# amaciarey/PathIntegralGroundState

Hardware: AMD Instinct MI355X
Metric: bead-pair action evals/sec (K1 Delta-S, N=256 Nb=161 4He, 128 walkers/GPU) (higher is better)
Workload: dtype f64; 1 GPU; liquid 4He N=256 beads=161 (namelist Nb=80), 128 walkers/GPU x 1 GPU(s) = 128 walkers, one full-chain Delta-S stage per step (20608 items x 255 partners per GPU); walkers_per_gpu=128, global_walkers=128

## Files before the change

### pathintegralgroundstate_amd/csrc/pigs_device.h

```cpp
#pragma once

#include <hip/hip_runtime.h>
#include <stdint.h>

namespace pigs {

constexpr int kWave = 64;

struct DevParams {
    int32_t dim, Np, NpPad, Nb;
    int32_t M, Nmax, trap, wf_table;
    int32_t v_table, nW, pad1, pad2;
    double  dr, rcut2, dt, Rm;
    double  Lbox[3], LboxHalf[3], a_ho[3];
    double  rdr;
    double  hrdr;
    double  rLbox[3];
};

__host__ __device__ inline size_t slice_doubles(int dim, int NpPad) { return (size_t)dim * NpPad; }

__device__ __forceinline__ double wave_sum(double v)
{
#pragma unroll
    for (int off = 32; off >= 1; off >>= 1) v += __shfl_xor(v, off, kWave);
    return v;
}

template <int DIM>
__device__ __forceinline__ double min_image(double (&x)[DIM], const DevParams &P)
{
    double r2 = 0.0;
#pragma unroll
    for (int k = 0; k < DIM; ++k) {
        double v = x[k];
        if (v >  P.LboxHalf[k]) v = v - P.Lbox[k];
        if (v < -P.LboxHalf[k]) v = v + P.Lbox[k];
        x[k] = v;
        r2 = r2 + v * v;
    }
    return r2;
}

template <int DIM>
__device__ __forceinline__ double plain_r2(const double (&x)[DIM])
{
    double r2 = 0.0;
#pragma unroll
    for (int k = 0; k < DIM; ++k) r2 = r2 + x[k] * x[k];
    return r2;
}

struct Lerp {
    int    ix;
    int    im2;
    double a1, a2;
};

__device__ __forceinline__ Lerp lerp_setup(double x, double dx, int Nmax)
{
    Lerp L;
    int ix = (int)(x / dx) + 1;
    L.a1   = x - (double)(ix - 1) * dx;
    L.a2   = dx - L.a1;
    L.ix   = min(ix, Nmax);
    L.im2  = max(L.ix - 2, 0);
    return L;
}

__device__ __forceinline__ double interp0(const double *__restrict__ F, const Lerp &L, double dx)
{
    return (L.a1 * F[L.ix] + L.a2 * F[L.ix - 1]) / dx;
}

__device__ __forceinline__ double interp1(const double *__restrict__ F, const Lerp &L, double dx)
{
    double Fbefore = (L.a1 * F[L.ix - 1] + L.a2 * F[L.im2]) / dx;
    double Fafter  = (L.a1 * F[L.ix + 1] + L.a2 * F[L.ix]) / dx;
    return 0.5 * (Fafter - Fbefore) / dx;
}

__device__ __forceinline__ double interp2(const double *__restrict__ F, const Lerp &L, double dx)
{
    double Fbefore = (L.a1 * F[L.ix - 1] + L.a2 * F[L.im2]) / dx;
    double Fcurr   = (L.a1 * F[L.ix] + L.a2 * F[L.ix - 1]) / dx;
    double Fafter  = (L.a1 * F[L.ix + 1] + L.a2 * F[L.ix]) / dx;
    return (Fafter - 2.0 * Fcurr + Fbefore) / (dx * dx);
}

__device__ __forceinline__ double div_by(double a, double d, double rd)
{
    const double q = a * rd;
    const double r = __builtin_fma(-q, d, a);
    return __builtin_fma(r, rd, q);
}

__device__ __forceinline__ double div_by_inf(double a, double d, double rd)
{
    const double q = a * rd;
    const double r = __builtin_fma(-q, d, a);
    const double z = __builtin_fma(r, rd, q);
    return __builtin_fabs(q) == __builtin_inf() ? q : z;
}

__device__ __forceinline__ void sqrt_rinv(double x, double &s, double &y)
{
    const double y0 = __builtin_amdgcn_rsq(x);
    double g = x * y0;
    double h = 0.5 * y0;
    const double r0 = __builtin_fma(-h, g, 0.5);
    g = __builtin_fma(g, r0, g);
    h = __builtin_fma(h, r0, h);
    const double d0 = __builtin_fma(-g, g, x);
    g = __builtin_fma(d0, h, g);
    const double d1 = __builtin_fma(-g, g, x);
    g = __builtin_fma(d1, h, g);
    s = g;
    double yy = h + h;
    const double e = __builtin_fma(-g, yy, 1.0);
    y = __builtin_fma(e, yy, yy);
}

__device__ __forceinline__ double sqrt_exact(double x)
{
    double s, y;
    sqrt_rinv(x, s, y);
    return s;
}

struct FLerp {
    int    ix, im2;
    double a1, a2;
};

__device__ __forceinline__ FLerp flerp_setup(double x, const DevParams &P)
{
    FLerp L;
    const int ix = (int)div_by(x, P.dr, P.rdr) + 1;
    L.a1  = x - (double)(ix - 1) * P.dr;
    L.a2  = P.dr - L.a1;
    L.ix  = min(ix, P.Nmax);
#ifdef PIGS_EXPERIMENT_HOT_TABLE
    L.ix  = (L.ix & 63) + 2;
#endif
    L.im2 = max(L.ix - 2, 0);
    return L;
}

template <typename TabPtr>
__device__ __forceinline__ double finterp0(TabPtr F, const FLerp &L, const DevParams &P)
{
    return div_by_inf(L.a1 * F[L.ix] + L.a2 * F[L.ix - 1], P.dr, P.rdr);
}

template <typename TabPtr>
__device__ __forceinline__ void finterp01(TabPtr F, const FLerp &L, const DevParams &P, double &v0, double &v1)
{
    const double fm2 = F[L.im2], fm1 = F[L.ix - 1], f0 = F[L.ix], fp1 = F[L.ix + 1];
    v0 = div_by_inf(L.a1 * f0 + L.a2 * fm1, P.dr, P.rdr);
    const double Fbefore = div_by_inf(L.a1 * fm1 + L.a2 * fm2, P.dr, P.rdr);
    const double Fafter  = div_by_inf(L.a1 * fp1 + L.a2 * f0, P.dr, P.rdr);
    v1 = div_by_inf(0.5 * (Fafter - Fbefore), P.dr, P.rdr);
}

template <int DIM>
__device__ __forceinline__ double min_image_fast(double (&x)[DIM], const DevParams &P)
{
    double r2 = 0.0;
#pragma unroll
    for (int k = 0; k < DIM; ++k) {
        const double v = x[k];
        const double w = v - __builtin_copysign(P.Lbox[k], v);
        const double u = (__builtin_fabs(v) > P.LboxHalf[k]) ? w : v;
        x[k] = u;
        r2 = r2 + u * u;
    }
    return r2;
}

struct FastTab {
    const double *p;
    __device__ __forceinline__ double operator[](int i) const { return p[i]; }
};
template <typename T> struct is_fast_tab { static constexpr bool value = false; };
template <> struct is_fast_tab<FastTab> { static constexpr bool value = true; };

template <int DIM>
__device__ __forceinline__ double min_image_rn(double (&x)[DIM], const DevParams &P)
{
    double r2 = 0.0;
#pragma unroll
    for (int k = 0; k < DIM; ++k) {
        const double v = x[k];
        const double t = __builtin_fmin(__builtin_fmax(__builtin_fabs(v) * P.rLbox[k], 0.0), 1.0);
        const double n = __builtin_copysign(__builtin_rint(t), v);
        const double u = __builtin_fma(-P.Lbox[k], n, v);
        x[k] = u;
        r2 = r2 + u * u;
    }
    return r2;
}

template <int DIM>
__device__ __forceinline__ double min_image_mag(const double (&x)[DIM], const DevParams &P)
{
    double r2 = 0.0;
#pragma unroll
    for (int k = 0; k < DIM; ++k) {
        const double a = __builtin_fabs(x[k]);
        const double m = __builtin_fmin(a, P.Lbox[k] - a);
        r2 = r2 + m * m;
    }
    return r2;
}

struct FCell {
    int    i0;
    double f, omf;
    double r, rinv;
};

__device__ __forceinline__ FCell fcell_setup(double r2, const DevParams &P)
{
    FCell C;
    const double y0 = __builtin_amdgcn_rsq(r2);
    double g = r2 * y0;
    double h = 0.5 * y0;
    const double r0 = __builtin_fma(-h, g, 0.5);
    g = __builtin_fma(g, r0, g);
    h = __builtin_fma(h, r0, h);
    const double d0 = __builtin_fma(-g, g, r2);
    g = __builtin_fma(d0, h, g);
    C.r    = g;
    C.rinv = h + h;
    const double t = g * P.rdr;
    C.i0  = (int)t;
    C.f   = t - (double)C.i0;
    C.omf = 1.0 - C.f;
    return C;
}

template <int N>
__device__ __forceinline__ void wave_reduce_multi(double (&v)[N], int lane)
{
    int stride = 32;
#pragma unroll
    for (int cnt = N; cnt > 1; cnt >>= 1, stride >>= 1) {
        const bool upper = (lane & stride) != 0;
#pragma unroll
        for (int i = 0; i < cnt / 2; ++i) {
            const double send = upper ? v[i] : v[i + cnt / 2];
            const double keep = upper ? v[i + cnt / 2] : v[i];
            v[i] = keep + __shfl_xor(send, stride, kWave);
        }
    }
#pragma unroll
    for (; stride >= 1; stride >>= 1) v[0] += __shfl_xor(v[0], stride, kWave);
}

constexpr int kRedStride = 65;

template <int N>
__device__ __forceinline__ double wave_reduce_lds(const double (&v)[N], double *scratch, int lane)
{
    static_assert(N == 2 || N == 4 || N == 8, "N must divide 64");
#pragma unroll
    for (int i = 0; i < N; ++i) scratch[i * kRedStride + lane] = v[i];
    __builtin_amdgcn_wave_barrier();
    const int vi = lane % N, g = lane / N;
    const double *row = scratch + vi * kRedStride + g * N;
    double s = row[0];
#pragma unroll
    for (int k = 1; k < N; ++k) s = s + row[k];
    __builtin_amdgcn_wave_barrier();
#pragma unroll
    for (int stride = N; stride < kWave; stride <<= 1) s = s + __shfl_xor(s, stride, kWave);
    return s;
}

template <int N>
__device__ __forceinline__ constexpr int lane_of(int i)
{
    int lane = 0, stride = 32;
    for (int cnt = N; cnt > 1; cnt >>= 1, stride >>= 1)
        if (i & (cnt >> 1)) lane |= stride;
    return lane;
}

__device__ __forceinline__ double read_lane(double v, int lane)
{
    union { double d; int i[2]; } u;
    u.d = v;
    u.i[0] = __builtin_amdgcn_readlane(u.i[0], lane);
    u.i[1] = __builtin_amdgcn_readlane(u.i[1], lane);
    return u.d;
}

template <int N>
__device__ __forceinline__ double row_shl(double x)
{
    union { double d; int i[2]; } u, r;
    u.d = x;
    r.i[0] = __builtin_amdgcn_update_dpp(0, u.i[0], 0x100 + N, 0xf, 0xf, true);
    r.i[1] = __builtin_amdgcn_update_dpp(0, u.i[1], 0x100 + N, 0xf, 0xf, true);
    return r.d;
}

__host__ __device__ inline double green_function(int opt, int ib, int Nb, double dt, double Pot, double F2)
{
    double g = 0.0;
    if (opt == 0) {
        double Ve = Pot;
        double Vc = Pot + dt * dt * F2 / 6.0;
        if (ib == 0 || ib == 2 * Nb) g = dt * Ve / 3.0;
        else if ((ib & 1) == 0)      g = 2.0 * dt * Ve / 3.0;
        else                         g = 4.0 * dt * Vc / 3.0;
    } else {
        double dVe = Pot;
        double dVc = Pot + dt * dt * F2 / 2.0;
        if (ib == 0 || ib == 2 * Nb) g = dVe / 3.0;
        else if ((ib & 1) == 0)      g = 2.0 * dVe / 3.0;
        else                         g = 4.0 * dVc / 3.0;
    }
    return g;
}

__device__ __forceinline__ double green_function_action(int ib, int Nb, double dt_in, double Pot, double F2)
{
    constexpr double r3 = 1.0 / 3.0, r6 = 1.0 / 6.0;
    double dt = dt_in;
    asm volatile("" : "+v"(dt));
    if (ib == 0 || ib == 2 * Nb) return div_by_inf(dt * Pot, 3.0, r3);
    if ((ib & 1) == 0)           return div_by_inf(2.0 * dt * Pot, 3.0, r3);
    const double Vc = Pot + div_by_inf(dt * dt * F2, 6.0, r6);
    return div_by_inf(4.0 * dt * Vc, 3.0, r3);
}

__host__ __device__ inline double log_psi(int opt, double Rm, double r)
{
    const double q = Rm / r;
    const double q5 = q * q * q * q * q;
    if (opt == 0) return -0.5 * q5;
    if (opt == 1) return 2.5 * q5 / r;
    return -15.0 * q5 / (r * r);
}

__host__ __device__ inline double trap_pot(int opt, double a, double x)
{
    const double a4 = a * a * a * a;
    return opt == 0 ? 0.5 * (x * x) / a4 : x / a4;
}

__host__ __device__ inline double trap_psi(int opt, double a, double x)
{
    if (opt == 0) { double q = x / a; return -0.5 * (q * q); }
    if (opt == 1) return -(x / (a * a));
    return -1.0 / (a * a);
}

}
```

### pathintegralgroundstate_amd/csrc/pigs_k1.hip

```cpp
#include <atomic>

#include "pigs_device.h"
#include "pigs_k1_device.h"
#include "pigs_kernels.h"

namespace pigs {

template <int DIM, bool TRAP>
__global__ __launch_bounds__(256) void k_delta_action_v1(
    DevParams P, const double *__restrict__ paths, const double *__restrict__ VT,
    const double *__restrict__ WF, int n_items, const int32_t *__restrict__ walker,
    const int32_t *__restrict__ ipv, const int32_t *__restrict__ ibv,
    const double *__restrict__ xnew, const double *__restrict__ xold,
    double *__restrict__ out, double *__restrict__ parts)
{
    const int lane  = threadIdx.x & (kWave - 1);
    const int wid   = threadIdx.x >> 6;
    const int nwave = gridDim.x * (blockDim.x >> 6);
    const size_t sl = slice_doubles(DIM, P.NpPad);

    for (int item = blockIdx.x * (blockDim.x >> 6) + wid; item < n_items; item += nwave) {
        const int it = __builtin_amdgcn_readfirstlane(item);
        const int w  = walker[it];
        const int p  = ipv[it] - 1;
        const int b  = ibv[it];
        if ((unsigned)w >= (unsigned)P.nW || (unsigned)p >= (unsigned)P.Np || (unsigned)b >= (unsigned)P.M) {
            if (lane == 0) out[it] = __builtin_nan("");
            continue;
        }
        double xn[DIM], xo[DIM];
#pragma unroll
        for (int k = 0; k < DIM; ++k) {
            xn[k] = xnew[(size_t)it * DIM + k];
            xo[k] = xold[(size_t)it * DIM + k];
        }
        const double *S   = paths + ((size_t)w * P.M + b) * sl;
        const bool odd    = (b & 1) != 0;
        const bool endb   = (b == 0) || (b == 2 * P.Nb);

        double potN = 0.0, potO = 0.0, psiN = 0.0, psiO = 0.0;
        double fN[DIM], fO[DIM];
#pragma unroll
        for (int k = 0; k < DIM; ++k) { fN[k] = 0.0; fO[k] = 0.0; }

        if (TRAP && lane == 0) {
#pragma unroll
            for (int k = 0; k < DIM; ++k) {
                potN = potN + trap_pot(0, P.a_ho[k], xn[k]);
                potO = potO + trap_pot(0, P.a_ho[k], xo[k]);
                fO[k] = trap_pot(1, P.a_ho[k], xo[k]);
                fN[k] = trap_pot(1, P.a_ho[k], xn[k]);
                if (endb) {
                    psiO = psiO + trap_psi(0, P.a_ho[k], xo[k]);
                    psiN = psiN + trap_psi(0, P.a_ho[k], xn[k]);
                }
            }
        }

        for (int j0 = 0; j0 < P.Np; j0 += kWave) {
            const int j = j0 + lane;
            if (j < P.Np && j != p) {
                double dnew[DIM], dold[DIM];
#pragma unroll
                for (int k = 0; k < DIM; ++k) {
                    const double rj = S[(size_t)k * P.NpPad + j];
                    dnew[k] = xn[k] - rj;
                    dold[k] = xo[k] - rj;
                }
                double r2n, r2o;
                if (TRAP) { r2o = plain_r2<DIM>(dold); r2n = plain_r2<DIM>(dnew); }
                else      { r2o = min_image<DIM>(dold, P); r2n = min_image<DIM>(dnew, P); }

                if (TRAP || r2n <= P.rcut2) {
                    const double r = sqrt(r2n);
                    const Lerp L = lerp_setup(r, P.dr, P.Nmax);
                    potN = potN + interp0(VT, L, P.dr);
                    if (odd) {
                        const double dv = interp1(VT, L, P.dr);
#pragma unroll
                        for (int k = 0; k < DIM; ++k) fN[k] = fN[k] + dv * dnew[k] / r;
                    }
                    if (endb) psiN = psiN + (P.wf_table ? interp0(WF, L, P.dr) : log_psi(0, P.Rm, r));
                }
                if (r2o <= P.rcut2) {
                    const double r = sqrt(r2o);
                    const Lerp L = lerp_setup(r, P.dr, P.Nmax);
                    potO = potO + interp0(VT, L, P.dr);
                    if (odd) {
                        const double dv = interp1(VT, L, P.dr);
#pragma unroll
                        for (int k = 0; k < DIM; ++k) fO[k] = fO[k] + dv * dold[k] / r;
                    }
                    if (endb) psiO = psiO + (P.wf_table ? interp0(WF, L, P.dr) : log_psi(0, P.Rm, r));
                } else if (TRAP && endb) {
                    const double r = sqrt(r2o);
                    const Lerp L = lerp_setup(r, P.dr, P.Nmax);
                    psiO = psiO + (P.wf_table ? interp0(WF, L, P.dr) : log_psi(0, P.Rm, r));
                }
            }
        }

        potN = wave_sum(potN);
        potO = wave_sum(potO);
        double dF2 = 0.0, dPsi = 0.0;
        if (odd) {
            double fn2 = 0.0, fo2 = 0.0;
#pragma unroll
            for (int k = 0; k < DIM; ++k) {
                const double a = wave_sum(fN[k]);
                const double c = wave_sum(fO[k]);
                fn2 = fn2 + a * a;
                fo2 = fo2 + c * c;
            }
            dF2 = fn2 - fo2;
        }
        if (endb) {
            psiN = wave_sum(psiN);
            psiO = wave_sum(psiO);
            dPsi = psiN - psiO;
        }
        if (lane == 0) {
            const double dPot = potN - potO;
            out[it] = -dPsi + green_function(0, b, P.Nb, P.dt, dPot, dF2);
            if (parts) {
                parts[(size_t)it * 3 + 0] = dPot;
                parts[(size_t)it * 3 + 1] = dF2;
                parts[(size_t)it * 3 + 2] = dPsi;
            }
        }
    }
}


template <int DIM, bool TRAP, int BLOCK, bool PREFETCH = false, bool FAST = false>
__global__ __launch_bounds__(BLOCK) void k_delta_action_v2(
    DevParams P, const double *__restrict__ paths, const double *__restrict__ VT,
    const double *__restrict__ WF, int n_items, const int32_t *__restrict__ walker,
    const int32_t *__restrict__ ipv, const int32_t *__restrict__ ibv,
    const double *__restrict__ xnew, const double *__restrict__ xold,
    double *__restrict__ out, double *__restrict__ parts)
{
    extern __shared__ __attribute__((aligned(16))) unsigned char smem[];
    const int lane  = threadIdx.x & (kWave - 1);
    const int wid   = threadIdx.x >> 6;
    const int nwave = gridDim.x * (BLOCK >> 6);
    const size_t sl = slice_doubles(DIM, P.NpPad);
    double *red = reinterpret_cast<double *>(smem + (size_t)wid * kWaveLds);

    for (int item = blockIdx.x * (BLOCK >> 6) + wid; item < n_items; item += nwave) {
        const int it = __builtin_amdgcn_readfirstlane(item);
        const int w  = walker[it];
        const int p  = ipv[it] - 1;
        const int b  = ibv[it];
        if ((unsigned)w >= (unsigned)P.nW || (unsigned)p >= (unsigned)P.Np || (unsigned)b >= (unsigned)P.M) {
            if (lane == 0) out[it] = __builtin_nan("");
            continue;
        }
        double xn[DIM], xo[DIM];
#pragma unroll
        for (int k = 0; k < DIM; ++k) {
            xn[k] = xnew[(size_t)it * DIM + k];
            xo[k] = xold[(size_t)it * DIM + k];
        }
        const double *S = paths + ((size_t)w * P.M + b) * sl;
        double *o = out + it;
        double *q = parts ? parts + (size_t)it * 3 : nullptr;
        if (FAST && !TRAP) {
            if (PREFETCH) item_eval_prefetch<DIM, TRAP>(P, FastTab{VT}, WF, S, p, b, xn, xo, lane, red, o, q);
            else          item_eval<DIM, TRAP>(P, FastTab{VT}, WF, S, p, b, xn, xo, lane, red, o, q);
        } else if (PREFETCH) {
            item_eval_prefetch<DIM, TRAP>(P, VT, WF, S, p, b, xn, xo, lane, red, o, q);
        } else {
            item_eval<DIM, TRAP>(P, VT, WF, S, p, b, xn, xo, lane, red, o, q);
        }
    }
}

template <int DIM>
__global__ __launch_bounds__(256) void k_delta_action_grid(
    DevParams P, const double *__restrict__ paths, const double *__restrict__ VTimg,
    const double *__restrict__ WF, int n_items, const int32_t *__restrict__ walker,
    const int32_t *__restrict__ ipv, const int32_t *__restrict__ ibv,
    const double *__restrict__ xnew, const double *__restrict__ xold,
    double *__restrict__ out, double *__restrict__ parts)
{
    extern __shared__ __attribute__((aligned(16))) unsigned char smem[];
    const int lane  = threadIdx.x & (kWave - 1);
    const int wid   = threadIdx.x >> 6;
    const int nwave = gridDim.x * 4;
    const size_t sl = slice_doubles(DIM, P.NpPad);
    double *red = reinterpret_cast<double *>(smem + (size_t)wid * kWaveLds);
    const PipeTab VT{VTimg + 2, P.Nmax + 3};

    for (int item = blockIdx.x * 4 + wid; item < n_items; item += nwave) {
        const int it = __builtin_amdgcn_readfirstlane(item);
        const int w  = walker[it];
        const int p  = ipv[it] - 1;
        const int b  = ibv[it];
        if ((unsigned)w >= (unsigned)P.nW || (unsigned)p >= (unsigned)P.Np || (unsigned)b >= (unsigned)P.M) {
            if (lane == 0) out[it] = __builtin_nan("");
            continue;
        }
        double xn[DIM], xo[DIM];
#pragma unroll
        for (int k = 0; k < DIM; ++k) {
            xn[k] = xnew[(size_t)it * DIM + k];
            xo[k] = xold[(size_t)it * DIM + k];
        }
        item_eval_pipe<DIM>(P, VT, WF, paths + ((size_t)w * P.M + b) * sl, p, b, xn, xo, lane, red, out + it,
                            parts ? parts + (size_t)it * 3 : nullptr);
    }
}

template <int DIM, bool TRAP, int CLS>
__device__ __forceinline__ void reforder_item(const DevParams &P, const double *__restrict__ VT, const double *__restrict__ WF,
                                              const double *__restrict__ S, int p, int b, const double (&xn)[DIM],
                                              const double (&xo)[DIM], int lane, double *T, double *out, double *parts)
{
    for (int j = lane; j < P.Np; j += kWave) {
        Acc<DIM, CLS> A;
        if (j != p) {
            double rj[DIM];
#pragma unroll
            for (int k = 0; k < DIM; ++k) rj[k] = S[(size_t)k * P.NpPad + j];
            partner_accumulate_at<DIM, TRAP, CLS>(P, VT, WF, rj, xn, xo, A);
        }
        double *t = T + (size_t)j * 8;
        t[0] = A.potN; t[1] = A.potO;
        if (CLS == CLS_ODD) {
#pragma unroll
            for (int k = 0; k < DIM; ++k) { t[2 + k] = A.fN[k]; t[5 + k] = A.fO[k]; }
        } else if (CLS == CLS_END) {
            t[2] = A.psiN; t[3] = A.psiO;
        }
    }
    __builtin_amdgcn_wave_barrier();
    __syncthreads();
    double s = 0.0;
    if (lane < 8) {
        if (TRAP) {
            Acc<DIM, CLS> A0;
            trap_terms<DIM, TRAP, CLS>(P, xn, xo, A0);
            double col[8] = {A0.potN, A0.potO, 0.0, 0.0, 0.0, 0.0, 0.0, 0.0};
            if (CLS == CLS_ODD) {
#pragma unroll
                for (int k = 0; k < DIM; ++k) { col[2 + k] = A0.fN[k]; col[5 + k] = A0.fO[k]; }
            } else if (CLS == CLS_END) {
                col[2] = A0.psiN; col[3] = A0.psiO;
            }
#pragma unroll
            for (int q = 0; q < 8; ++q) if (lane == q) s = col[q];
        }
        for (int j = 0; j < P.Np; ++j) {
            if (j == p) continue;
            s = s + T[(size_t)j * 8 + lane];
        }
    }
    const double c0 = read_lane(s, 0), c1 = read_lane(s, 1);
    double dF2 = 0.0, dPsi = 0.0;
    if (CLS == CLS_ODD) {
        double fn2 = 0.0, fo2 = 0.0;
#pragma unroll
        for (int k = 0; k < DIM; ++k) {
            const double a = read_lane(s, 2 + k), c = read_lane(s, 5 + k);
            fn2 = fn2 + a * a;
            fo2 = fo2 + c * c;
        }
        dF2 = fn2 - fo2;
    } else if (CLS == CLS_END) {
        dPsi = read_lane(s, 2) - read_lane(s, 3);
    }
    const double dPot = c0 - c1;
    if (lane == 0) {
        *out = -dPsi + green_function(0, b, P.Nb, P.dt, dPot, dF2);
        if (parts) { parts[0] = dPot; parts[1] = dF2; parts[2] = dPsi; }
    }
}

template <int DIM, bool TRAP>
__global__ __launch_bounds__(64) void k_delta_action_reforder(
    DevParams P, const double *__restrict__ paths, const double *__restrict__ VT,
    const double *__restrict__ WF, int n_items, const int32_t *__restrict__ walker,
    const int32_t *__restrict__ ipv, const int32_t *__restrict__ ibv,
    const double *__restrict__ xnew, const double *__restrict__ xold,
    double *__restrict__ out, double *__restrict__ parts)
{
    extern __shared__ __attribute__((aligned(16))) unsigned char smem[];
    double *T = reinterpret_cast<double *>(smem);
    const int lane = threadIdx.x;
    const size_t sl = slice_doubles(DIM, P.NpPad);
    for (int it = blockIdx.x; it < n_items; it += gridDim.x) {
        const int w = walker[it], p = ipv[it] - 1, b = ibv[it];
        if ((unsigned)w >= (unsigned)P.nW || (unsigned)p >= (unsigned)P.Np || (unsigned)b >= (unsigned)P.M) {
            if (lane == 0) out[it] = __builtin_nan("");
            continue;
        }
        double xn[DIM], xo[DIM];
#pragma unroll
        for (int k = 0; k < DIM; ++k) {
            xn[k] = xnew[(size_t)it * DIM + k];
            xo[k] = xold[(size_t)it * DIM + k];
        }
        const double *S = paths + ((size_t)w * P.M + b) * sl;
        double *o = out + it;
        double *q = parts ? parts + (size_t)it * 3 : nullptr;
        const bool odd  = (b & 1) != 0;
        const bool endb = (b == 0) || (b == 2 * P.Nb);
        if (odd)       reforder_item<DIM, TRAP, CLS_ODD>(P, VT, WF, S, p, b, xn, xo, lane, T, o, q);
        else if (endb) reforder_item<DIM, TRAP, CLS_END>(P, VT, WF, S, p, b, xn, xo, lane, T, o, q);
        else           reforder_item<DIM, TRAP, CLS_EVEN>(P, VT, WF, S, p, b, xn, xo, lane, T, o, q);
        __syncthreads();
    }
}

__device__ __forceinline__ size_t pipe_tab_bytes(int nt) { return ((size_t)(nt + 6) * sizeof(double) + 15) & ~(size_t)15; }


__device__ __forceinline__ void pipe_table_dma_issue(unsigned char *smem, const double *__restrict__ VTg, int nt, int wid, int lane)
{
#ifndef PIGS_EXPERIMENT_NO_STAGE
    const double2 *src = reinterpret_cast<const double2 *>(VTg);
    const int n2 = nt / 2;
    for (int cb = wid * kWave; cb < n2; cb += (int)blockDim.x) {
        const int idx = cb + lane;
        auto *l = reinterpret_cast<__attribute__((address_space(3))) void *>(
            (__attribute__((address_space(3))) unsigned char *)smem + 16 + (size_t)cb * 16);
        if (idx < n2) __builtin_amdgcn_global_load_lds((const __attribute__((address_space(1))) void *)(src + idx), l, 16, 0, 0);
    }
#endif
}

__device__ __forceinline__ PipeTab pipe_table_dma_finish(unsigned char *smem, const double *__restrict__ VTg, int nt)
{
    double *base = reinterpret_cast<double *>(smem);
    double *tab  = base + 2;
    asm volatile("s_waitcnt vmcnt(0)" ::: "memory");
    if (threadIdx.x == 0) {
        if (nt & 1) tab[nt - 1] = VTg[nt - 1];
        base[0] = 0.0; base[1] = tab[0];
        tab[nt] = 0.0; tab[nt + 1] = 0.0; tab[nt + 2] = 0.0; tab[nt + 3] = 0.0;
    }
    return PipeTab{tab, nt + 1};
}

template <int DIM>
struct ItemMeta {
    int    p, b, ok;
    const double *S;
    double xn[DIM], xo[DIM];
};

struct ItemRaw {
    int    i;
    double x;
};

template <int DIM>
__device__ __forceinline__ ItemRaw pipe2_request(int it, const int32_t *__restrict__ walker,
                                                 const int32_t *__restrict__ ipv, const int32_t *__restrict__ ibv,
                                                 const double *__restrict__ xnew, const double *__restrict__ xold, int lane)
{
    ItemRaw r;
    const int32_t *ai = lane == 0 ? walker : (lane == 1 ? ipv : ibv);
    r.i = ai[it];
    const int k = lane < DIM ? lane : (lane < 2 * DIM ? lane - DIM : 0);
    const double *ax = lane < DIM ? xnew : xold;
    r.x = ax[(size_t)it * DIM + k];
    return r;
}

__device__ __forceinline__ double bcast_lane(double v, int lane_id)
{
    union { double d; int i[2]; } u;
    u.d = v;
    u.i[0] = __builtin_amdgcn_readlane(u.i[0], lane_id);
    u.i[1] = __builtin_amdgcn_readlane(u.i[1], lane_id);
    return u.d;
}

template <int DIM>
__device__ __forceinline__ void pipe2_decode(const DevParams &P, const double *__restrict__ paths, const ItemRaw &r,
                                             size_t sl, ItemMeta<DIM> &R)
{
    const int w = __builtin_amdgcn_readlane(r.i, 0);
    R.p = __builtin_amdgcn_readlane(r.i, 1) - 1;
    R.b = __builtin_amdgcn_readlane(r.i, 2);
    R.ok = (unsigned)w < (unsigned)P.nW && (unsigned)R.p < (unsigned)P.Np && (unsigned)R.b < (unsigned)P.M;
#pragma unroll
    for (int k = 0; k < DIM; ++k) {
        R.xn[k] = bcast_lane(r.x, k);
        R.xo[k] = bcast_lane(r.x, DIM + k);
    }
    R.S = paths + (R.ok ? ((size_t)w * P.M + R.b) * sl : 0);
}

template <int DIM>
__device__ __forceinline__ const double *pipe2_slice(const DevParams &P, const double *__restrict__ paths, const ItemRaw &r, size_t sl)
{
    const int w = __builtin_amdgcn_readlane(r.i, 0);
    const int p = __builtin_amdgcn_readlane(r.i, 1) - 1;
    const int b = __builtin_amdgcn_readlane(r.i, 2);
    const bool ok = (unsigned)w < (unsigned)P.nW && (unsigned)p < (unsigned)P.Np && (unsigned)b < (unsigned)P.M;
    return paths + (ok ? ((size_t)w * P.M + b) * sl : 0);
}

template <int DIM>
__device__ __forceinline__ void pipe2_load(const DevParams &P, const double *__restrict__ S, int p, int m, int lane,
                                           double (&rj)[DIM])
{
    const int j  = m * kWave + lane;
    const int jj = pipe_row(P, j, p);
#pragma unroll
    for (int k = 0; k < DIM; ++k) rj[k] = S[(size_t)k * P.NpPad + jj];
}

template <int DIM, int CLS, int M>
__device__ __forceinline__ void pipe2_pass(const DevParams &P, PipeTab VT, const double *__restrict__ WF,
                                           const ItemMeta<DIM> &R, const double (&rjm)[DIM], int lane, Acc<DIM, CLS> &A)
{
    const int j = M * kWave + lane;
    const bool valid = j < P.Np && j != R.p;
    double dn[DIM], dold[DIM];
#pragma unroll
    for (int k = 0; k < DIM; ++k) {
        double rj = rjm[k];
        asm volatile("; class %1 pass %2" : "+v"(rj) : "n"(CLS), "n"(M));
        dn[k] = R.xn[k] - rj; dold[k] = R.xo[k] - rj;
    }
    const double r2o = pipe_r2<DIM, CLS>(dold, P);
    const double r2n = pipe_r2<DIM, CLS>(dn, P);
    pipe_pair<DIM, CLS, false>(P, VT, WF, floor_r2(r2n), valid && r2n <= P.rcut2, dn, A);
    pipe_pair<DIM, CLS, true>(P, VT, WF, floor_r2(r2o), valid && r2o <= P.rcut2, dold, A);
    __builtin_amdgcn_sched_barrier(0);
}

template <int DIM>
struct PipeState {
    ItemRaw raw_next;
    ItemRaw raw_nn;
    int k_nn;
    bool has_next;
    const double *idle;
    double a0[DIM], a1[DIM];
};

template <int DIM, int CLS>
__device__ __forceinline__ void pipe2_item(const DevParams &P, PipeTab VT, const double *__restrict__ WF,
                                           const double *__restrict__ paths, size_t sl, int n_local, int *queue,
                                           const int32_t *__restrict__ walker, const int32_t *__restrict__ ipv,
                                           const int32_t *__restrict__ ibv, const double *__restrict__ xnew,
                                           const double *__restrict__ xold,
                                           const ItemMeta<DIM> &R, PipeState<DIM> &st, int k_self, int lane, double *red,
                                           double *out, double *parts)
{
    Acc<DIM, CLS> A;
    double b0[DIM], b1[DIM];
    pipe2_load<DIM>(P, R.S, R.p, 2, lane, b0);
    pipe2_pass<DIM, CLS, 0>(P, VT, WF, R, st.a0, lane, A);
    pipe2_load<DIM>(P, R.S, R.p, 3, lane, b1);
    pipe2_pass<DIM, CLS, 1>(P, VT, WF, R, st.a1, lane, A);
    const double *Snext = st.has_next ? pipe2_slice<DIM>(P, paths, st.raw_next, sl) : st.idle;
    {
        int kn = 0;
        if (lane == 0) kn = atomicAdd(queue, 1);
        kn = __builtin_amdgcn_readfirstlane(kn);
        st.k_nn = kn;
        const int kq = kn < n_local ? kn : k_self;
        st.raw_nn = pipe2_request<DIM>((int)blockIdx.x + kq * (int)gridDim.x, walker, ipv, ibv, xnew, xold, lane);
    }
    const int pnext = __builtin_amdgcn_readlane(st.raw_next.i, 1) - 1;
    pipe2_load<DIM>(P, Snext, pnext, 0, lane, st.a0);
    pipe2_pass<DIM, CLS, 2>(P, VT, WF, R, b0, lane, A);
    pipe2_load<DIM>(P, Snext, pnext, 1, lane, st.a1);
    pipe2_pass<DIM, CLS, 3>(P, VT, WF, R, b1, lane, A);
    finish_item<DIM, CLS>(P, lane, R.b, A, red, out, parts);
}

#ifdef PIGS_EXPERIMENT_K1_CLOCK
constexpr int kK1ClockWaves = 16 * 1024;
__device__ unsigned long long k1_clock[kK1ClockWaves * 5];
#define K1STAMP(v) const unsigned long long v = __builtin_amdgcn_s_memrealtime()
#else
#define K1STAMP(v) do { } while (0)
#endif

template <int DIM>
__global__ __launch_bounds__(1024) void k_delta_action_pipe2(
    DevParams P, const double *__restrict__ paths, const double *__restrict__ VTg,
    const double *__restrict__ WF, int n_items, const int32_t *__restrict__ walker,
    const int32_t *__restrict__ ipv, const int32_t *__restrict__ ibv,
    const double *__restrict__ xnew, const double *__restrict__ xold,
    double *__restrict__ out, double *__restrict__ parts)
{
    extern __shared__ __attribute__((aligned(16))) unsigned char smem[];
    __shared__ int next_local;
    const int lane  = threadIdx.x & (kWave - 1);
    const int wid   = __builtin_amdgcn_readfirstlane(threadIdx.x >> 6);
    const size_t sl = slice_doubles(DIM, P.NpPad);
    const int n_local = (n_items - (int)blockIdx.x + (int)gridDim.x - 1) / (int)gridDim.x;

    int k_cur = wid, k_nx = wid + 16;
    ItemMeta<DIM> cur;
    PipeState<DIM> st;
    const int nt = P.Nmax + 2;
    K1STAMP(t_entry);
    pipe_table_dma_issue(smem, VTg, nt, wid, lane);
    {
        const ItemRaw r0 = pipe2_request<DIM>((int)blockIdx.x + (k_cur < n_local ? k_cur : 0) * (int)gridDim.x,
                                              walker, ipv, ibv, xnew, xold, lane);
        st.raw_next = pipe2_request<DIM>((int)blockIdx.x + (k_nx < n_local ? k_nx : (k_cur < n_local ? k_cur : 0)) * (int)gridDim.x,
                                         walker, ipv, ibv, xnew, xold, lane);
        pipe2_decode<DIM>(P, paths, r0, sl, cur);
        pipe2_load<DIM>(P, cur.S, cur.p, 0, lane, st.a0);
        pipe2_load<DIM>(P, cur.S, cur.p, 1, lane, st.a1);
    }

    const PipeTab VT = pipe_table_dma_finish(smem, VTg, nt);
    K1STAMP(t_loaded);
    if (threadIdx.x == 0) next_local = 32;
    double *red = reinterpret_cast<double *>(smem + pipe_tab_bytes(nt) + (size_t)wid * kWaveLds);
    __syncthreads();
    K1STAMP(t_ready);
#ifdef PIGS_EXPERIMENT_K1_CLOCK
    int n_done = 0;
#endif

    st.idle = (size_t)(P.Nmax + 2) >= sl ? VTg : paths;
    while (k_cur < n_local) {
        st.has_next = k_nx < n_local;
        const int it = (int)blockIdx.x + k_cur * (int)gridDim.x;
        double *o = out + it;
        double *q = nullptr;
        if (!cur.ok) {
            if (lane == 0) *o = __builtin_nan("");
            const double *Snext = st.has_next ? pipe2_slice<DIM>(P, paths, st.raw_next, sl) : st.idle;
            int kn = 0;
            if (lane == 0) kn = atomicAdd(&next_local, 1);
            kn = __builtin_amdgcn_readfirstlane(kn);
            st.k_nn = kn;
            st.raw_nn = pipe2_request<DIM>((int)blockIdx.x + (kn < n_local ? kn : k_cur) * (int)gridDim.x,
                                           walker, ipv, ibv, xnew, xold, lane);
            const int pnext = __builtin_amdgcn_readlane(st.raw_next.i, 1) - 1;
            pipe2_load<DIM>(P, Snext, pnext, 0, lane, st.a0);
            pipe2_load<DIM>(P, Snext, pnext, 1, lane, st.a1);
        } else {
            const bool odd  = (cur.b & 1) != 0;
            const bool endb = (cur.b == 0) || (cur.b == 2 * P.Nb);
            if (odd)       pipe2_item<DIM, CLS_ODD>(P, VT, WF, paths, sl, n_local, &next_local, walker, ipv, ibv, xnew, xold, cur, st, k_cur, lane, red, o, q);
            else if (endb) pipe2_item<DIM, CLS_END>(P, VT, WF, paths, sl, n_local, &next_local, walker, ipv, ibv, xnew, xold, cur, st, k_cur, lane, red, o, q);
            else           pipe2_item<DIM, CLS_EVEN>(P, VT, WF, paths, sl, n_local, &next_local, walker, ipv, ibv, xnew, xold, cur, st, k_cur, lane, red, o, q);
        }
        pipe2_decode<DIM>(P, paths, st.raw_next, sl, cur);
        k_cur = k_nx;
        k_nx = st.k_nn;
        st.raw_next = st.raw_nn;
#ifdef PIGS_EXPERIMENT_K1_CLOCK
        ++n_done;
#endif
    }
#ifdef PIGS_EXPERIMENT_K1_CLOCK
    K1STAMP(t_end);
    const int slot = (int)blockIdx.x * 16 + wid;
    if (lane == 0 && slot < kK1ClockWaves) {
        unsigned long long *c = k1_clock + (size_t)slot * 5;
        c[0] = t_entry; c[1] = t_loaded; c[2] = t_ready; c[3] = t_end; c[4] = (unsigned long long)n_done;
    }
#endif
}

__global__ void k_selftest_fastmath(DevParams P, unsigned long long seed, int iters, unsigned long long *bad)
{
    unsigned long long s = seed ^ (0x9E3779B97F4A7C15ull * (blockIdx.x * (unsigned long long)blockDim.x + threadIdx.x + 1));
    unsigned long long b0 = 0, b1 = 0, b2 = 0, b3 = 0;
    for (int i = 0; i < iters; ++i) {
        s ^= s << 13; s ^= s >> 7; s ^= s << 17;
        const double u1 = (double)(s >> 11) * (1.0 / 9007199254740992.0);
        s ^= s << 13; s ^= s >> 7; s ^= s << 17;
        const double u2 = (double)(s >> 11) * (1.0 / 9007199254740992.0);
        const double rmax2 = 4.0 * P.rcut2;
        const double x = (i & 1) ? u1 * rmax2 : u1 * u1 * 1e-3 + 1e-12;
        double sq, y;
        sqrt_rinv(x, sq, y);
        if (sq != sqrt(x)) ++b0;
        const double num = (u2 - 0.5) * ((i & 2) ? 1e6 : 3.0);
        if (div_by(num, sq, y) != num / sq) ++b1;
        if (div_by(sq, P.dr, P.rdr) != sq / P.dr) ++b2;
        if (div_by(num, P.dr, P.rdr) != num / P.dr) ++b3;
    }
    atomicAdd(&bad[0], b0); atomicAdd(&bad[1], b1); atomicAdd(&bad[2], b2); atomicAdd(&bad[3], b3);
}

#define PIGS_DISPATCH(P, CALL)                                              \
    do {                                                                    \
        if ((P).trap) {                                                     \
            if ((P).dim == 1) { CALL(1, true); }                            \
            else if ((P).dim == 2) { CALL(2, true); }                       \
            else { CALL(3, true); }                                         \
        } else {                                                            \
            if ((P).dim == 1) { CALL(1, false); }                           \
            else if ((P).dim == 2) { CALL(2, false); }                      \
            else { CALL(3, false); }                                        \
        }                                                                   \
    } while (0)

static int k1_grid(int n_items, int waves_per_block, int cap_blocks)
{
    int blocks = (n_items + waves_per_block - 1) / waves_per_block;
    return blocks < cap_blocks ? (blocks > 0 ? blocks : 1) : cap_blocks;
}

static int k1_pipe_blocks()
{
    static int n = 0;
    if (n == 0) {
        int dev = 0;
        hipDeviceProp_t pr;
        if (hipGetDevice(&dev) == hipSuccess && hipGetDeviceProperties(&pr, dev) == hipSuccess && pr.multiProcessorCount > 0)
            n = pr.multiProcessorCount;
        else
            n = 256;
    }
    return n;
}

template <auto Kern>
static hipError_t set_lds(size_t bytes)
{
    if (bytes <= 64 * 1024) return hipSuccess;
    constexpr int kMaxDev = 64;
    static std::atomic<size_t> granted[kMaxDev];
    int dev = 0;
    if (hipGetDevice(&dev) != hipSuccess || dev < 0 || dev >= kMaxDev) dev = -1;
    if (dev >= 0 && bytes <= granted[dev].load(std::memory_order_acquire)) return hipSuccess;
    const hipError_t e = hipFuncSetAttribute(reinterpret_cast<const void *>(Kern), hipFuncAttributeMaxDynamicSharedMemorySize, (int)bytes);
    if (e == hipSuccess && dev >= 0) {
        size_t g = granted[dev].load(std::memory_order_relaxed);
        while (g < bytes && !granted[dev].compare_exchange_weak(g, bytes, std::memory_order_release)) {}
    }
    return e;
}

hipError_t launch_delta_action(const DevParams &P, int variant, const double *paths, const double *VT,
                               const double *VTimg, const double *WF, int n_items, const int32_t *walker,
                               const int32_t *ip, const int32_t *ib, const double *xnew,
                               const double *xold, double *out, double *parts, hipStream_t st)
{
    if (n_items <= 0) return hipSuccess;
    const size_t pipe_bytes = (((size_t)(P.Nmax + 2 + 6) * sizeof(double)) + 15) & ~(size_t)15;
    const bool can_pipe = !P.trap && P.Np <= 256 && VTimg && pipe_bytes + 16 * kWaveLds <= 160 * 1024;
    if (variant == K1_AUTO) {
        if (P.trap) variant = K1_V2;
        else if (can_pipe) variant = (n_items >= 16 * k1_pipe_blocks() && !parts) ? K1_PIPE2 : K1_GRID;
        else variant = K1_FAST;
    }
    if ((variant == K1_PIPE2 || variant == K1_GRID) && !can_pipe) variant = P.trap ? K1_V2 : K1_FAST;
    if (variant == K1_PIPE2 && parts) variant = K1_GRID;
    if (variant == K1_FAST_PREFETCH && P.Np > 256) variant = K1_FAST;
    if ((variant == K1_FAST || variant == K1_FAST_PREFETCH) && P.trap) variant = K1_V2;
    hipError_t e = hipSuccess;
    switch (variant) {
    case K1_V1: {
#define CALL(D, T)                                                                              \
    hipLaunchKernelGGL((k_delta_action_v1<D, T>), dim3(k1_grid(n_items, 4, 2048)), dim3(256), 0, st, P, \
                       paths, VT, WF, n_items, walker, ip, ib, xnew, xold, out, parts)
        PIGS_DISPATCH(P, CALL);
#undef CALL
        break;
    }
    case K1_V2:
    case K1_FAST:
    case K1_FAST_PREFETCH: {
        const size_t lds = 4 * kWaveLds;
        const int grid = k1_grid(n_items, 4, 1 << 22);
#define CALL(D, T)                                                                                             \
    do {                                                                                                       \
        if (variant == K1_V2)                                                                                  \
            hipLaunchKernelGGL((k_delta_action_v2<D, T, 256, false, false>), dim3(grid), dim3(256), lds, st, P, \
                               paths, VT, WF, n_items, walker, ip, ib, xnew, xold, out, parts);                \
        else if (variant == K1_FAST)                                                                           \
            hipLaunchKernelGGL((k_delta_action_v2<D, T, 256, false, true>), dim3(grid), dim3(256), lds, st, P, \
                               paths, VT, WF, n_items, walker, ip, ib, xnew, xold, out, parts);                \
        else                                                                                                   \
            hipLaunchKernelGGL((k_delta_action_v2<D, T, 256, true, true>), dim3(grid), dim3(256), lds, st, P,  \
                               paths, VT, WF, n_items, walker, ip, ib, xnew, xold, out, parts);                \
    } while (0)
        PIGS_DISPATCH(P, CALL);
#undef CALL
        break;
    }
    case K1_GRID: {
        const size_t lds = 4 * kWaveLds;
        const int grid = k1_grid(n_items, 4, 1 << 22);
#define CALLP(D)                                                                                        \
    hipLaunchKernelGGL((k_delta_action_grid<D>), dim3(grid), dim3(256), lds, st, P, paths, VTimg, WF,   \
                       n_items, walker, ip, ib, xnew, xold, out, parts)
        if (P.dim == 1) CALLP(1); else if (P.dim == 2) CALLP(2); else CALLP(3);
#undef CALLP
        break;
    }
    case K1_PIPE2: {
        const size_t lds = pipe_bytes + 16 * kWaveLds;
        int blocks = (n_items + 15) / 16;
        if (blocks > k1_pipe_blocks()) blocks = k1_pipe_blocks();
#define CALLP(D)                                                                                        \
    do {                                                                                                \
        e = set_lds<k_delta_action_pipe2<D>>(lds);                                                      \
        if (e == hipSuccess)                                                                            \
            hipLaunchKernelGGL((k_delta_action_pipe2<D>), dim3(blocks), dim3(1024), lds, st, P, paths,  \
                               VT, WF, n_items, walker, ip, ib, xnew, xold, out, parts);                \
    } while (0)
        if (P.dim == 1) CALLP(1); else if (P.dim == 2) CALLP(2); else CALLP(3);
#undef CALLP
        break;
    }
    case K1_REFORDER: {
        const size_t lds = (size_t)P.Np * 8 * sizeof(double);
        if (lds > 160 * 1024) return hipErrorInvalidValue;
        const int grid = n_items < (1 << 16) ? n_items : (1 << 16);
#define CALL(D, T)                                                                                      \
    do {                                                                                                \
        e = set_lds<k_delta_action_reforder<D, T>>(lds);                                                \
        if (e == hipSuccess)                                                                            \
            hipLaunchKernelGGL((k_delta_action_reforder<D, T>), dim3(grid), dim3(64), lds, st, P, paths, VT, WF, \
                               n_items, walker, ip, ib, xnew, xold, out, parts);                        \
    } while (0)
        PIGS_DISPATCH(P, CALL);
#undef CALL
        break;
    }
    default:
        return hipErrorInvalidValue;
    }
    if (e != hipSuccess) return e;
    return hipGetLastError();
}

#ifdef PIGS_EXPERIMENT_K1_CLOCK
extern "C" int pigs_k1_clock_read(unsigned long long *dst, int n_waves)
{
    if (!dst || n_waves <= 0 || n_waves > kK1ClockWaves) return -1;
    if (hipDeviceSynchronize() != hipSuccess) return -1;
    return hipMemcpyFromSymbol(dst, HIP_SYMBOL(k1_clock), (size_t)n_waves * 5 * sizeof(unsigned long long), 0,
                               hipMemcpyDeviceToHost) == hipSuccess ? 0 : -1;
}
#endif

hipError_t launch_selftest_fastmath(const DevParams &P, unsigned long long seed, int blocks, int iters,
                                    unsigned long long *d_bad, hipStream_t st)
{
    hipLaunchKernelGGL(k_selftest_fastmath, dim3(blocks), dim3(256), 0, st, P, seed, iters, d_bad);
    return hipGetLastError();
}

}
```

Measured before the change: 187.3 billion bead-pair action evals/s.

## Use buffer loads with out-of-range self-row masking and swizzle-based wave reductions

Replaces the per-lane pipe_row index remap for partner coordinate loads with raw buffer loads. The self-particle lane gets a huge offset, so the hardware bounds check returns zero, and invalid or idle slices get a zero-sized range. The table DMA wait now leaves the initial partner loads in flight (vmcnt(2*DIM)), and the table tail is read up front. The cross-lane reduction steps switch from shfl_xor to ds_swizzle and permlane32_swap. All of this aims to cut address ALU work, the idle-pointer logic and LDS-based shuffle latency, but it depends on zero-fill semantics from out-of-bounds buffer loads and on the vmcnt ordering being correct.

```diff
diff --git a/pathintegralgroundstate_amd/csrc/pigs_device.h b/pathintegralgroundstate_amd/csrc/pigs_device.h
--- a/pathintegralgroundstate_amd/csrc/pigs_device.h
+++ b/pathintegralgroundstate_amd/csrc/pigs_device.h
@@ -258,6 +258,25 @@
     for (; stride >= 1; stride >>= 1) v[0] += __shfl_xor(v[0], stride, kWave);
 }
 
+template <int S>
+__device__ __forceinline__ double add_xor_lane(double s)
+{
+    union { double d; int i[2]; } u, a, b;
+    u.d = s;
+    if constexpr (S < 32) {
+        a.i[0] = __builtin_amdgcn_ds_swizzle(u.i[0], (S << 10) | 0x1f);
+        a.i[1] = __builtin_amdgcn_ds_swizzle(u.i[1], (S << 10) | 0x1f);
+        return s + a.d;
+    } else {
+        static_assert(S == 32, "xor stride must be a power of two below 64");
+        const auto lo = __builtin_amdgcn_permlane32_swap(u.i[0], u.i[0], false, false);
+        const auto hi = __builtin_amdgcn_permlane32_swap(u.i[1], u.i[1], false, false);
+        a.i[0] = lo[0]; a.i[1] = hi[0];
+        b.i[0] = lo[1]; b.i[1] = hi[1];
+        return a.d + b.d;
+    }
+}
+
 constexpr int kRedStride = 65;
 
 template <int N>
@@ -273,8 +292,11 @@
 #pragma unroll
     for (int k = 1; k < N; ++k) s = s + row[k];
     __builtin_amdgcn_wave_barrier();
-#pragma unroll
-    for (int stride = N; stride < kWave; stride <<= 1) s = s + __shfl_xor(s, stride, kWave);
+    if constexpr (N <= 2) s = add_xor_lane<2>(s);
+    if constexpr (N <= 4) s = add_xor_lane<4>(s);
+    s = add_xor_lane<8>(s);
+    s = add_xor_lane<16>(s);
+    s = add_xor_lane<32>(s);
     return s;
 }
 
diff --git a/pathintegralgroundstate_amd/csrc/pigs_k1.hip b/pathintegralgroundstate_amd/csrc/pigs_k1.hip
--- a/pathintegralgroundstate_amd/csrc/pigs_k1.hip
+++ b/pathintegralgroundstate_amd/csrc/pigs_k1.hip
@@ -330,13 +330,14 @@
 #endif
 }
 
-__device__ __forceinline__ PipeTab pipe_table_dma_finish(unsigned char *smem, const double *__restrict__ VTg, int nt)
+template <int IN_FLIGHT>
+__device__ __forceinline__ PipeTab pipe_table_dma_finish(unsigned char *smem, int nt, double tail)
 {
     double *base = reinterpret_cast<double *>(smem);
     double *tab  = base + 2;
-    asm volatile("s_waitcnt vmcnt(0)" ::: "memory");
+    asm volatile("s_waitcnt vmcnt(%0)" :: "n"(IN_FLIGHT) : "memory");
     if (threadIdx.x == 0) {
-        if (nt & 1) tab[nt - 1] = VTg[nt - 1];
+        if (nt & 1) tab[nt - 1] = tail;
         base[0] = 0.0; base[1] = tab[0];
         tab[nt] = 0.0; tab[nt + 1] = 0.0; tab[nt + 2] = 0.0; tab[nt + 3] = 0.0;
     }
@@ -347,6 +348,7 @@
 struct ItemMeta {
     int    p, b, ok;
     const double *S;
+    int    nb;
     double xn[DIM], xo[DIM];
 };
 
@@ -392,26 +394,36 @@
         R.xo[k] = bcast_lane(r.x, DIM + k);
     }
     R.S = paths + (R.ok ? ((size_t)w * P.M + R.b) * sl : 0);
-}
-
-template <int DIM>
-__device__ __forceinline__ const double *pipe2_slice(const DevParams &P, const double *__restrict__ paths, const ItemRaw &r, size_t sl)
+    R.nb = R.ok ? P.NpPad * 8 : 0;
+}
+
+struct SliceRef {
+    const double *S;
+    int nb;
+};
+
+__device__ __forceinline__ SliceRef pipe2_slice(const DevParams &P, const double *__restrict__ paths, const ItemRaw &r,
+                                                size_t sl, bool has)
 {
     const int w = __builtin_amdgcn_readlane(r.i, 0);
     const int p = __builtin_amdgcn_readlane(r.i, 1) - 1;
     const int b = __builtin_amdgcn_readlane(r.i, 2);
-    const bool ok = (unsigned)w < (unsigned)P.nW && (unsigned)p < (unsigned)P.Np && (unsigned)b < (unsigned)P.M;
-    return paths + (ok ? ((size_t)w * P.M + b) * sl : 0);
-}
+    const bool ok = has && (unsigned)w < (unsigned)P.nW && (unsigned)p < (unsigned)P.Np && (unsigned)b < (unsigned)P.M;
+    return SliceRef{paths + (ok ? ((size_t)w * P.M + b) * sl : 0), ok ? P.NpPad * 8 : 0};
+}
+
+constexpr unsigned kPipeRowOff = 0x40000000u;
 
 template <int DIM>
-__device__ __forceinline__ void pipe2_load(const DevParams &P, const double *__restrict__ S, int p, int m, int lane,
-                                           double (&rj)[DIM])
-{
-    const int j  = m * kWave + lane;
-    const int jj = pipe_row(P, j, p);
-#pragma unroll
-    for (int k = 0; k < DIM; ++k) rj[k] = S[(size_t)k * P.NpPad + jj];
+__device__ __forceinline__ void pipe2_load(const DevParams &P, const double *__restrict__ S, int nbytes, int p, int m,
+                                           int lane, double (&rj)[DIM])
+{
+    const unsigned off = (lane == p - m * kWave ? kPipeRowOff : (unsigned)lane * 8u) + (unsigned)(m * kWave * 8);
+#pragma unroll
+    for (int k = 0; k < DIM; ++k) {
+        const auto rs = __builtin_amdgcn_make_buffer_rsrc(const_cast<double *>(S + (size_t)k * P.NpPad), 0, nbytes, 0x00020000);
+        rj[k] = __builtin_bit_cast(double, __builtin_amdgcn_raw_buffer_load_b64(rs, off, 0, 0));
+    }
 }
 
 template <int DIM, int CLS, int M>
@@ -440,7 +452,6 @@
     ItemRaw raw_nn;
     int k_nn;
     bool has_next;
-    const double *idle;
     double a0[DIM], a1[DIM];
 };
 
@@ -455,11 +466,11 @@
 {
     Acc<DIM, CLS> A;
     double b0[DIM], b1[DIM];
-    pipe2_load<DIM>(P, R.S, R.p, 2, lane, b0);
+    pipe2_load<DIM>(P, R.S, R.nb, R.p, 2, lane, b0);
     pipe2_pass<DIM, CLS, 0>(P, VT, WF, R, st.a0, lane, A);
-    pipe2_load<DIM>(P, R.S, R.p, 3, lane, b1);
+    pipe2_load<DIM>(P, R.S, R.nb, R.p, 3, lane, b1);
     pipe2_pass<DIM, CLS, 1>(P, VT, WF, R, st.a1, lane, A);
-    const double *Snext = st.has_next ? pipe2_slice<DIM>(P, paths, st.raw_next, sl) : st.idle;
+    const SliceRef Snext = pipe2_slice(P, paths, st.raw_next, sl, st.has_next);
     {
         int kn = 0;
         if (lane == 0) kn = atomicAdd(queue, 1);
@@ -469,9 +480,9 @@
         st.raw_nn = pipe2_request<DIM>((int)blockIdx.x + kq * (int)gridDim.x, walker, ipv, ibv, xnew, xold, lane);
     }
     const int pnext = __builtin_amdgcn_readlane(st.raw_next.i, 1) - 1;
-    pipe2_load<DIM>(P, Snext, pnext, 0, lane, st.a0);
+    pipe2_load<DIM>(P, Snext.S, Snext.nb, pnext, 0, lane, st.a0);
     pipe2_pass<DIM, CLS, 2>(P, VT, WF, R, b0, lane, A);
-    pipe2_load<DIM>(P, Snext, pnext, 1, lane, st.a1);
+    pipe2_load<DIM>(P, Snext.S, Snext.nb, pnext, 1, lane, st.a1);
     pipe2_pass<DIM, CLS, 3>(P, VT, WF, R, b1, lane, A);
     finish_item<DIM, CLS>(P, lane, R.b, A, red, out, parts);
 }
@@ -505,17 +516,18 @@
     const int nt = P.Nmax + 2;
     K1STAMP(t_entry);
     pipe_table_dma_issue(smem, VTg, nt, wid, lane);
+    const double tail = VTg[nt - 1];
     {
         const ItemRaw r0 = pipe2_request<DIM>((int)blockIdx.x + (k_cur < n_local ? k_cur : 0) * (int)gridDim.x,
                                               walker, ipv, ibv, xnew, xold, lane);
         st.raw_next = pipe2_request<DIM>((int)blockIdx.x + (k_nx < n_local ? k_nx : (k_cur < n_local ? k_cur : 0)) * (int)gridDim.x,
                                          walker, ipv, ibv, xnew, xold, lane);
         pipe2_decode<DIM>(P, paths, r0, sl, cur);
-        pipe2_load<DIM>(P, cur.S, cur.p, 0, lane, st.a0);
-        pipe2_load<DIM>(P, cur.S, cur.p, 1, lane, st.a1);
-    }
-
-    const PipeTab VT = pipe_table_dma_finish(smem, VTg, nt);
+        pipe2_load<DIM>(P, cur.S, cur.nb, cur.p, 0, lane, st.a0);
+        pipe2_load<DIM>(P, cur.S, cur.nb, cur.p, 1, lane, st.a1);
+    }
+
+    const PipeTab VT = pipe_table_dma_finish<2 * DIM>(smem, nt, tail);
     K1STAMP(t_loaded);
     if (threadIdx.x == 0) next_local = 32;
     double *red = reinterpret_cast<double *>(smem + pipe_tab_bytes(nt) + (size_t)wid * kWaveLds);
@@ -525,7 +537,6 @@
     int n_done = 0;
 #endif
 
-    st.idle = (size_t)(P.Nmax + 2) >= sl ? VTg : paths;
     while (k_cur < n_local) {
         st.has_next = k_nx < n_local;
         const int it = (int)blockIdx.x + k_cur * (int)gridDim.x;
@@ -533,7 +544,7 @@
         double *q = nullptr;
         if (!cur.ok) {
             if (lane == 0) *o = __builtin_nan("");
-            const double *Snext = st.has_next ? pipe2_slice<DIM>(P, paths, st.raw_next, sl) : st.idle;
+            const SliceRef Snext = pipe2_slice(P, paths, st.raw_next, sl, st.has_next);
             int kn = 0;
             if (lane == 0) kn = atomicAdd(&next_local, 1);
             kn = __builtin_amdgcn_readfirstlane(kn);
@@ -541,8 +552,8 @@
             st.raw_nn = pipe2_request<DIM>((int)blockIdx.x + (kn < n_local ? kn : k_cur) * (int)gridDim.x,
                                            walker, ipv, ibv, xnew, xold, lane);
             const int pnext = __builtin_amdgcn_readlane(st.raw_next.i, 1) - 1;
-            pipe2_load<DIM>(P, Snext, pnext, 0, lane, st.a0);
-            pipe2_load<DIM>(P, Snext, pnext, 1, lane, st.a1);
+            pipe2_load<DIM>(P, Snext.S, Snext.nb, pnext, 0, lane, st.a0);
+            pipe2_load<DIM>(P, Snext.S, Snext.nb, pnext, 1, lane, st.a1);
         } else {
             const bool odd  = (cur.b & 1) != 0;
             const bool endb = (cur.b == 0) || (cur.b == 2 * P.Nb);
```

Measured after the change: 193.9 billion bead-pair action evals/s, median of 6. 3.5% higher.
